# tayloraswift/jpeg

Measured on AMD Instinct MI355X. Metric: Mpixels/s decode (IDCT+dequant+upsample+YCbCr->RGB); % HBM roofline, higher is better.
Workload: dtype f32; 1 GPU; C3: one 8192x8192 ycc8 4:2:0 image per GPU per step, fused Spectral->RGB8 decode (ring of 4 distinct images); sampling=4:2:0, output=RGB8, coefficients=distribution N (SURVEY 8d), seeded, quanta=CompressionLevel luminance/chrominance(1.0), parallelism=independent images x1 (weak scaling), no data-path collective

## Files before the change

include/jpeg_amd.h:

```cpp
#ifndef JPEG_AMD_H
#define JPEG_AMD_H

#include <stddef.h>
#include <stdint.h>

#ifdef __cplusplus
extern "C" {
#endif

#define JPEG_AMD_VERSION 100
#define JPEG_AMD_MAX_PLANES 4

typedef enum jpeg_amd_status {
    JPEG_AMD_OK      = 0,
    JPEG_AMD_EINVAL  = -1,
    JPEG_AMD_ENOMEM  = -2,
    JPEG_AMD_EHIP    = -3,
    JPEG_AMD_ENODEV  = -4,
    JPEG_AMD_ENOSUP  = -5
} jpeg_amd_status;

typedef struct jpeg_amd_ctx jpeg_amd_ctx;

typedef struct jpeg_amd_layout {
// ... 5 lines not shown
    int32_t factor_y[JPEG_AMD_MAX_PLANES];
    int32_t units_x[JPEG_AMD_MAX_PLANES];
    int32_t units_y[JPEG_AMD_MAX_PLANES];
    int32_t qi[JPEG_AMD_MAX_PLANES];
} jpeg_amd_layout;

typedef enum jpeg_amd_color {
    JPEG_AMD_COLOR_YCC8 = 0,
    JPEG_AMD_COLOR_RGB8 = 1
} jpeg_amd_color;

int         jpeg_amd_version(void);
const char *jpeg_amd_strerror(int status);
int         jpeg_amd_device_count(int *count);
#define JPEG_AMD_CTX_OWN_STREAM 1
int         jpeg_amd_ctx_create(int device, void *stream, int flags, jpeg_amd_ctx **ctx);
int         jpeg_amd_ctx_destroy(jpeg_amd_ctx *ctx);
int         jpeg_amd_ctx_synchronize(jpeg_amd_ctx *ctx);
int         jpeg_amd_last_hip_error(const jpeg_amd_ctx *ctx);
int         jpeg_amd_layout_units(jpeg_amd_layout *layout);

int jpeg_amd_malloc(jpeg_amd_ctx *ctx, size_t bytes, void **d_ptr);
int jpeg_amd_free(jpeg_amd_ctx *ctx, void *d_ptr);
int jpeg_amd_memcpy_h2d(jpeg_amd_ctx *ctx, void *d_dst, const void *h_src, size_t bytes);
int jpeg_amd_memcpy_d2h(jpeg_amd_ctx *ctx, void *h_dst, const void *d_src, size_t bytes);
int jpeg_amd_timer_begin(jpeg_amd_ctx *ctx);
int jpeg_amd_timer_end(jpeg_amd_ctx *ctx, float *elapsed_ms);


int jpeg_amd_idct_plane(jpeg_amd_ctx *ctx, const int16_t *d_coef, int units_x, int units_y,
                        const uint16_t h_quanta_zigzag[64], int precision,
                        uint16_t *d_plane);

int jpeg_amd_spectral_idct(jpeg_amd_ctx *ctx, const jpeg_amd_layout *layout,
// ... 257 lines not shown
```

jpeg_amd/_lib.py:

```python
from __future__ import annotations

import ctypes as C
import os

HERE = os.path.dirname(os.path.abspath(__file__))
LIB_PATH = os.environ.get("JPEG_AMD_LIBRARY") or os.path.join(HERE, "libjpeg_amd.so")
MAX_PLANES = 4

OK, EINVAL, ENOMEM, EHIP, ENODEV, ENOSUP = 0, -1, -2, -3, -4, -5
COLOR_YCC8, COLOR_RGB8 = 0, 1
CTX_OWN_STREAM = 1


class JpegAmdError(RuntimeError):
    def __init__(self, status: int, what: str, hip: int = 0):
        self.status, self.hip = status, hip
        msg = lib().jpeg_amd_strerror(status).decode()
        super().__init__(f"{what}: {msg} (status {status}" + (f", hipError {hip})" if hip else ")"))


class Layout(C.Structure):
    _fields_ = [
        ("width", C.c_int32), ("height", C.c_int32), ("precision", C.c_int32),
        ("nplanes", C.c_int32), ("scale_x", C.c_int32), ("scale_y", C.c_int32),
        ("factor_x", C.c_int32 * MAX_PLANES), ("factor_y", C.c_int32 * MAX_PLANES),
        ("units_x", C.c_int32 * MAX_PLANES), ("units_y", C.c_int32 * MAX_PLANES),
# ... 2 lines not shown


_p = C.c_void_p
_pp = C.POINTER(C.c_void_p)
_szp = C.POINTER(C.c_size_t)
_L = C.POINTER(Layout)

SIGNATURES = {
    "jpeg_amd_version": (C.c_int, []),
    "jpeg_amd_strerror": (C.c_char_p, [C.c_int]),
    "jpeg_amd_device_count": (C.c_int, [C.POINTER(C.c_int)]),
    "jpeg_amd_ctx_create": (C.c_int, [C.c_int, _p, C.c_int, _pp]),
    "jpeg_amd_ctx_destroy": (C.c_int, [_p]),
    "jpeg_amd_ctx_synchronize": (C.c_int, [_p]),
    "jpeg_amd_last_hip_error": (C.c_int, [_p]),
    "jpeg_amd_layout_units": (C.c_int, [_L]),
    "jpeg_amd_malloc": (C.c_int, [_p, C.c_size_t, _pp]),
    "jpeg_amd_free": (C.c_int, [_p, _p]),
    "jpeg_amd_memcpy_h2d": (C.c_int, [_p, _p, _p, C.c_size_t]),
    "jpeg_amd_memcpy_d2h": (C.c_int, [_p, _p, _p, C.c_size_t]),
    "jpeg_amd_timer_begin": (C.c_int, [_p]),
    "jpeg_amd_timer_end": (C.c_int, [_p, C.POINTER(C.c_float)]),
    "jpeg_amd_idct_plane": (C.c_int, [_p, _p, C.c_int, C.c_int, _p, C.c_int, _p]),
    "jpeg_amd_spectral_idct": (C.c_int, [_p, _L, _pp, _p, C.c_int, _pp]),
    "jpeg_amd_planar_interleaved": (C.c_int, [_p, _L, _pp, C.c_int, _p]),
    "jpeg_amd_rectangular_unpack": (C.c_int, [_p, _p, C.c_size_t, C.c_int, C.c_int, _p]),
    "jpeg_amd_decode_batch": (C.c_int, [_p, _L, C.c_int, _pp, _szp, _p, C.c_size_t, C.c_int,
                                        C.c_int, C.c_int, _p, C.c_size_t]),
    "jpeg_amd_decode": (C.c_int, [_p, _L, _pp, _p, C.c_int, C.c_int, C.c_int, _p]),
    "jpeg_amd_spectral_rectangular_batch": (C.c_int, [_p, _L, C.c_int, _pp, _szp, _p, C.c_size_t, C.c_int, C.c_int, _p, C.c_size_t]),
# ... 138 lines not shown
```

jpeg_amd/api.py:

```python
from __future__ import annotations

import ctypes as C
from dataclasses import dataclass
from typing import Dict, List, Optional, Sequence, Tuple

import numpy as np

from . import _lib

MAX_PLANES = _lib.MAX_PLANES


class YCbCr:
    code = _lib.COLOR_YCC8


class RGB:
    code = _lib.COLOR_RGB8


def _torch():
    import torch
    return torch


class Context:

    def __init__(self, device: int = 0, stream: Optional[int] = None, own_stream: bool = False):
        torch = _torch()
        if not torch.cuda.is_available():
            raise RuntimeError("jpeg_amd needs a GPU: torch.cuda.is_available() is False "
                               "(there is no CPU fallback)")
        self.device = int(device)
        self.torch_device = torch.device("cuda", self.device)
        if stream is None:
            stream = torch.cuda.current_stream(self.torch_device).cuda_stream
        self._h = C.c_void_p()
        flags = _lib.CTX_OWN_STREAM if own_stream else 0
        _lib.check(_lib.lib().jpeg_amd_ctx_create(self.device, C.c_void_p(stream), flags,
                                                 C.byref(self._h)), "jpeg_amd_ctx_create")

    @property
    def handle(self):
        return self._h

    def synchronize(self):
        _lib.check(_lib.lib().jpeg_amd_ctx_synchronize(self._h), "synchronize", self._h)

    def timer_begin(self):
        _lib.check(_lib.lib().jpeg_amd_timer_begin(self._h), "timer_begin", self._h)

    def timer_end(self) -> float:
        ms = C.c_float()
        _lib.check(_lib.lib().jpeg_amd_timer_end(self._h, C.byref(ms)), "timer_end", self._h)
        return ms.value

    def empty(self, n: int, dtype):
        torch = _torch()
        return torch.empty(max(int(n), 0), dtype=dtype, device=self.torch_device)

    def upload(self, a: np.ndarray):
        torch = _torch()
# ... 700 lines not shown
```

jpeg_amd/csrc/capi.hip:

```cpp
#pragma clang fp contract(off)

#include <hip/hip_runtime.h>

#include <cstdio>
#include <cstdlib>
#include <cstring>
#include <new>
#include <algorithm>
#include <atomic>
#include <memory>
#include <chrono>
#include <system_error>
#include <thread>
#include <vector>

#include "interleave.hpp"
#include "kernels.hpp"
#include "transform.hpp"
#include "worker_pool.hpp"

using namespace jpeg_amd;

struct jpeg_amd_ctx {
    int device = 0;
    hipStream_t stream = nullptr;
    bool own_stream = false;
    hipEvent_t ev_begin = nullptr, ev_end = nullptr;
    void *scratch = nullptr;
    size_t scratch_bytes = 0;
    uint16_t *d_qstage = nullptr;
    uint32_t *d_walk = nullptr;
    int32_t *d_flag = nullptr;
    void *d_region = nullptr;
    size_t region_bytes = 0;
    int qslot = 0;
    int last_hip = 0;
    void *file_pinned[2] = {nullptr, nullptr};
    void *file_device = nullptr;
    size_t file_pinned_bytes = 0, file_device_bytes = 0;
    hipEvent_t file_done[2] = {nullptr, nullptr};
    hipEvent_t file_decoded[2] = {nullptr, nullptr};
// ... 22 lines not shown
    catch (...) { return JPEG_AMD_ENOMEM; }

#define JA_TRY(expr)                          \
    do {                                      \
        const int s_ = (expr);                \
        if (s_ != JPEG_AMD_OK) return s_;     \
    } while (0)

int bind(jpeg_amd_ctx *ctx)
{
    if (!ctx) return JPEG_AMD_EINVAL;
    JA_HIP(ctx, hipSetDevice(ctx->device));
    return JPEG_AMD_OK;
}

int units_of(int size, int stride) { return size / stride + (size % stride != 0 ? 1 : 0); }

int check_layout(const jpeg_amd_layout *L, int ntables)
{
    if (!L) return JPEG_AMD_EINVAL;
    if (L->width <= 0 || L->height <= 0) return JPEG_AMD_EINVAL;
    if (L->precision < 1 || L->precision > 16) return JPEG_AMD_EINVAL;
    if (L->nplanes < 1 || L->nplanes > JPEG_AMD_MAX_PLANES) return JPEG_AMD_EINVAL;
    if (L->scale_x < 1 || L->scale_y < 1) return JPEG_AMD_EINVAL;
    for (int p = 0; p < L->nplanes; ++p) {
        if (L->factor_x[p] < 1 || L->factor_y[p] < 1) return JPEG_AMD_EINVAL;
        if (L->factor_x[p] > L->scale_x || L->factor_y[p] > L->scale_y) return JPEG_AMD_EINVAL;
        if (L->units_x[p] < 0 || L->units_y[p] < 0) return JPEG_AMD_EINVAL;
        if ((long long)L->units_x[p] * L->units_y[p] > (1LL << 30)) return JPEG_AMD_EINVAL;
        if (ntables >= 0 && (L->qi[p] < 0 || L->qi[p] >= ntables)) return JPEG_AMD_EINVAL;
// ... 13 lines not shown
            if (ix >= 8LL * L->units_x[p] || iy >= 8LL * L->units_y[p]) return JPEG_AMD_EINVAL;
        }
    }
    return JPEG_AMD_OK;
}

size_t plane_samples(const jpeg_amd_layout *L, int p)
{
    return (size_t)64 * L->units_x[p] * L->units_y[p];
}

int ensure_scratch(jpeg_amd_ctx *ctx, size_t bytes)
{
    if (bytes <= ctx->scratch_bytes) return JPEG_AMD_OK;
    if (ctx->scratch) {
        JA_HIP(ctx, hipStreamSynchronize(ctx->stream));
        JA_HIP(ctx, hipFree(ctx->scratch));
        ctx->scratch = nullptr;
        ctx->scratch_bytes = 0;
    }
    const size_t want = bytes + bytes / 8 + 4096;
    JA_HIP(ctx, hipMalloc(&ctx->scratch, want));
    ctx->scratch_bytes = want;
    return JPEG_AMD_OK;
}

int stage_quanta(jpeg_amd_ctx *ctx, const uint16_t *h_quanta, int ntables, const uint16_t **d_out)
{
    if (!h_quanta || ntables < 1 || ntables > JPEG_AMD_MAX_PLANES) return JPEG_AMD_EINVAL;
    uint16_t *slot = ctx->d_qstage + (size_t)ctx->qslot * kQSlotElems;
    ctx->qslot = (ctx->qslot + 1) % kQSlots;
// ... 118 lines not shown
struct SparseBudget {
    size_t blocks, arena, elems;
    bool ok;
};
SparseBudget sparse_budget(const jpeg_amd_layout &L)
{
    size_t blocks = 0;
    for (int c = 0; c < L.nplanes; ++c) blocks += (size_t)L.units_x[c] * L.units_y[c];
    const size_t arena = 24 * blocks;
    return {blocks, arena, blocks + arena, blocks + arena < 0xffffffffull};
}

int ensure_file_staging(jpeg_amd_ctx *ctx, size_t slot_bytes)
{
    if (ctx->file_pinned_bytes < slot_bytes) {
        JA_HIP(ctx, hipStreamSynchronize(ctx->stream));
        for (int i = 0; i < 2; ++i) {
            if (ctx->file_pinned[i]) { (void)hipHostFree(ctx->file_pinned[i]); ctx->file_pinned[i] = nullptr; }
            ctx->file_pinned_bytes = 0;
            JA_HIP(ctx, hipHostMalloc(&ctx->file_pinned[i], slot_bytes, hipHostMallocDefault));
            if (!ctx->file_done[i]) JA_HIP(ctx, hipEventCreateWithFlags(&ctx->file_done[i], hipEventDisableTiming));
            if (!ctx->file_decoded[i]) JA_HIP(ctx, hipEventCreateWithFlags(&ctx->file_decoded[i], hipEventDisableTiming));
            if (!ctx->file_fetched[i]) JA_HIP(ctx, hipEventCreateWithFlags(&ctx->file_fetched[i], hipEventDisableTiming));
        }
        ctx->file_pinned_bytes = slot_bytes;
    }
    if (!ctx->file_d2h) JA_HIP(ctx, hipStreamCreateWithFlags(&ctx->file_d2h, hipStreamNonBlocking));
    if (ctx->file_device_bytes < 2 * slot_bytes) {
        JA_HIP(ctx, hipStreamSynchronize(ctx->stream));
        JA_HIP(ctx, hipStreamSynchronize(ctx->file_d2h));
        if (ctx->file_device) { (void)hipFree(ctx->file_device); ctx->file_device = nullptr; ctx->file_device_bytes = 0; }
        JA_HIP(ctx, hipMalloc(&ctx->file_device, 2 * slot_bytes));
        ctx->file_device_bytes = 2 * slot_bytes;
    }
    return JPEG_AMD_OK;
}

int default_host_threads()
{
    int n = (int)std::max(1u, std::thread::hardware_concurrency());
    auto read_two = [](const char *path, long long &a, long long &b) -> bool {
        FILE *f = std::fopen(path, "r");
        if (!f) return false;
        char first[32] = {0};
// ... 82 lines not shown
    if (!ctx) return JPEG_AMD_ENOMEM;
    ctx->device = device;
    int status = JPEG_AMD_OK;
    do {
        if (hipSetDevice(device) != hipSuccess) { status = JPEG_AMD_ENODEV; break; }
        if (flags & JPEG_AMD_CTX_OWN_STREAM) {
            if (hipStreamCreateWithFlags(&ctx->stream, hipStreamNonBlocking) != hipSuccess) { status = JPEG_AMD_EHIP; break; }
            ctx->own_stream = true;
        } else {
            ctx->stream = static_cast<hipStream_t>(stream);
        }
        if (hipEventCreate(&ctx->ev_begin) != hipSuccess || hipEventCreate(&ctx->ev_end) != hipSuccess) { status = JPEG_AMD_EHIP; break; }
        if (hipMalloc(reinterpret_cast<void **>(&ctx->d_qstage), kQSlots * kQSlotElems * sizeof(uint16_t)) != hipSuccess) { status = JPEG_AMD_ENOMEM; break; }
        if (hipMalloc(reinterpret_cast<void **>(&ctx->d_walk), 256) != hipSuccess) { status = JPEG_AMD_ENOMEM; break; }
        if (hipMemset(ctx->d_walk, 0, 256) != hipSuccess) { status = JPEG_AMD_EHIP; break; }
    } while (0);
    if (status != JPEG_AMD_OK) {
        jpeg_amd_ctx_destroy(ctx);
        return status;
    }
    *out = ctx;
    return JPEG_AMD_OK;
}

int jpeg_amd_ctx_destroy(jpeg_amd_ctx *ctx)
{
    if (!ctx) return JPEG_AMD_OK;
    (void)hipSetDevice(ctx->device);
    (void)hipStreamSynchronize(ctx->stream);
    ctx->workers.reset();
    ctx->copiers.reset();
    if (ctx->scratch) (void)hipFree(ctx->scratch);
    if (ctx->d_region) (void)hipFree(ctx->d_region);
    if (ctx->d_qstage) (void)hipFree(ctx->d_qstage);
    if (ctx->d_walk) (void)hipFree(ctx->d_walk);
    if (ctx->d_flag) (void)hipFree(ctx->d_flag);
    for (int i = 0; i < 2; ++i) {
        if (ctx->file_pinned[i]) (void)hipHostFree(ctx->file_pinned[i]);
        if (ctx->file_done[i]) (void)hipEventDestroy(ctx->file_done[i]);
        if (ctx->file_decoded[i]) (void)hipEventDestroy(ctx->file_decoded[i]);
        if (ctx->file_fetched[i]) (void)hipEventDestroy(ctx->file_fetched[i]);
    }
    if (ctx->file_d2h) (void)hipStreamDestroy(ctx->file_d2h);
    if (ctx->file_device) (void)hipFree(ctx->file_device);
    if (ctx->ev_begin) (void)hipEventDestroy(ctx->ev_begin);
    if (ctx->ev_end) (void)hipEventDestroy(ctx->ev_end);
    if (ctx->own_stream && ctx->stream) (void)hipStreamDestroy(ctx->stream);
    delete ctx;
    return JPEG_AMD_OK;
}

int jpeg_amd_ctx_synchronize(jpeg_amd_ctx *ctx)
{
    JA_TRY(bind(ctx));
    JA_HIP(ctx, hipStreamSynchronize(ctx->stream));
    return JPEG_AMD_OK;
}

int jpeg_amd_last_hip_error(const jpeg_amd_ctx *ctx) { return ctx ? ctx->last_hip : 0; }

int jpeg_amd_layout_units(jpeg_amd_layout *L)
{
    if (!L || L->nplanes < 1 || L->nplanes > JPEG_AMD_MAX_PLANES || L->scale_x < 1 ||
        L->scale_y < 1 || L->width <= 0 || L->height <= 0)
        return JPEG_AMD_EINVAL;
    for (int p = 0; p < L->nplanes; ++p) {
        if (L->factor_x[p] < 1 || L->factor_y[p] < 1) return JPEG_AMD_EINVAL;
        L->units_x[p] = units_of(L->width * L->factor_x[p], 8 * L->scale_x);
        L->units_y[p] = units_of(L->height * L->factor_y[p], 8 * L->scale_y);
    }
    return JPEG_AMD_OK;
}


int jpeg_amd_malloc(jpeg_amd_ctx *ctx, size_t bytes, void **d_ptr)
{
    JA_TRY(bind(ctx));
    if (!d_ptr) return JPEG_AMD_EINVAL;
    *d_ptr = nullptr;
    if (bytes == 0) return JPEG_AMD_OK;
    JA_HIP(ctx, hipMalloc(d_ptr, bytes));
    return JPEG_AMD_OK;
}

int jpeg_amd_free(jpeg_amd_ctx *ctx, void *d_ptr)
{
    JA_TRY(bind(ctx));
    if (!d_ptr) return JPEG_AMD_OK;
    JA_HIP(ctx, hipStreamSynchronize(ctx->stream));
    JA_HIP(ctx, hipFree(d_ptr));
    return JPEG_AMD_OK;
}

int jpeg_amd_memcpy_h2d(jpeg_amd_ctx *ctx, void *d_dst, const void *h_src, size_t bytes)
{
    JA_TRY(bind(ctx));
    if (bytes == 0) return JPEG_AMD_OK;
    if (!d_dst || !h_src) return JPEG_AMD_EINVAL;
    JA_HIP(ctx, hipMemcpyAsync(d_dst, h_src, bytes, hipMemcpyHostToDevice, ctx->stream));
    JA_HIP(ctx, hipStreamSynchronize(ctx->stream));
    return JPEG_AMD_OK;
}

int jpeg_amd_memcpy_d2h(jpeg_amd_ctx *ctx, void *h_dst, const void *d_src, size_t bytes)
{
    JA_TRY(bind(ctx));
    if (bytes == 0) return JPEG_AMD_OK;
    if (!h_dst || !d_src) return JPEG_AMD_EINVAL;
    JA_HIP(ctx, hipMemcpyAsync(h_dst, d_src, bytes, hipMemcpyDeviceToHost, ctx->stream));
    JA_HIP(ctx, hipStreamSynchronize(ctx->stream));
    return JPEG_AMD_OK;
}

int jpeg_amd_timer_begin(jpeg_amd_ctx *ctx)
{
    JA_TRY(bind(ctx));
    JA_HIP(ctx, hipEventRecord(ctx->ev_begin, ctx->stream));
    return JPEG_AMD_OK;
}

int jpeg_amd_timer_end(jpeg_amd_ctx *ctx, float *elapsed_ms)
{
    JA_TRY(bind(ctx));
    if (!elapsed_ms) return JPEG_AMD_EINVAL;
    JA_HIP(ctx, hipEventRecord(ctx->ev_end, ctx->stream));
// ... 76 lines not shown
                          const uint16_t *d_quanta, size_t quanta_stride, int ntables,
                          int cosited, jpeg_amd_color color, uint8_t *d_pixels,
                          size_t pixel_stride)
{
    JA_TRY(bind(ctx));
    JA_TRY(check_layout(L, ntables));
    JA_TRY(check_planes_cover_image(L));
    JA_TRY(check_batch8(L, n_images, color));
    if (n_images == 0) return JPEG_AMD_OK;
    if (!d_coef || !coef_stride || !d_quanta || !d_pixels) return JPEG_AMD_EINVAL;
    PlaneSet cs;
    JA_TRY(plane_set(L, d_coef, coef_stride, true, &cs));
    const QuantaRef q{d_quanta, quanta_stride};
    const bool rgb = color == JPEG_AMD_COLOR_RGB8;
    if (fused_decode_supported(*L, cosited != 0)) {
        JA_HIP(ctx, launch_fused_decode(ctx->stream, n_images, *L, cs, q, rgb, ctx->d_walk, d_pixels, pixel_stride));
        return JPEG_AMD_OK;
    }
    return staged_decode(ctx, L, n_images, cs, q, cosited != 0, true, rgb ? PixelKind::RGB8 : PixelKind::YCC8, d_pixels, pixel_stride);
}

int jpeg_amd_decode(jpeg_amd_ctx *ctx, const jpeg_amd_layout *L, const int16_t *const d_coef[],
                    const uint16_t *h_quanta, int ntables, int cosited, jpeg_amd_color color,
                    uint8_t *d_pixels)
{
    JA_TRY(bind(ctx));
    JA_TRY(check_layout(L, ntables));
    const uint16_t *d_q = nullptr;
    JA_TRY(stage_quanta(ctx, h_quanta, ntables, &d_q));
    const size_t zero[JPEG_AMD_MAX_PLANES] = {0, 0, 0, 0};
    return jpeg_amd_decode_batch(ctx, L, 1, d_coef, zero, d_q, 0, ntables, cosited, color,
// ... 16 lines not shown

int stage_regions(jpeg_amd_ctx *ctx, const jpeg_amd_region *h, int n, const int32_t **d_regions, const uint32_t **d_tiles,
                  uint32_t *nwg)
{
    const size_t bytes = (size_t)16 * n + 4 * ((size_t)n + 1);
    std::vector<uint32_t> buf(bytes / 4);
    uint32_t acc = 0;
    for (int i = 0; i < n; ++i) {
        std::memcpy(&buf[4 * (size_t)i], &h[i], 16);
        buf[4 * (size_t)n + i] = acc;
        acc += region_tiles(h[i]);
    }
    buf[4 * (size_t)n + n] = acc;
    if (bytes > ctx->region_bytes) {
        if (ctx->d_region) {
            JA_HIP(ctx, hipStreamSynchronize(ctx->stream));
            JA_HIP(ctx, hipFree(ctx->d_region));
            ctx->d_region = nullptr;
            ctx->region_bytes = 0;
        }
        const size_t want = bytes + bytes / 8 + 4096;
        JA_HIP(ctx, hipMalloc(&ctx->d_region, want));
        ctx->region_bytes = want;
    }
    JA_HIP(ctx, hipMemcpyAsync(ctx->d_region, buf.data(), bytes, hipMemcpyHostToDevice, ctx->stream));
    *d_regions = static_cast<const int32_t *>(ctx->d_region);
    *d_tiles = reinterpret_cast<const uint32_t *>(static_cast<const int32_t *>(ctx->d_region) + 4 * (size_t)n);
    *nwg = acc;
    return JPEG_AMD_OK;
}

// ... 378 lines not shown
    const uint16_t *d_q = nullptr;
    JA_TRY(stage_quanta(ctx, h_quanta, ntables, &d_q));
    const size_t zero[JPEG_AMD_MAX_PLANES] = {0, 0, 0, 0};
    return jpeg_amd_encode_batch(ctx, L, 1, d_pixels, 0, color, d_q, 0, ntables, d_coef, zero);
}


namespace {

struct DeviceBag {
    jpeg_amd_ctx *ctx;
    std::vector<void *> ptrs;
    explicit DeviceBag(jpeg_amd_ctx *c) : ctx(c) {}
    ~DeviceBag()
    {
        (void)hipStreamSynchronize(ctx->stream);
        for (void *p : ptrs) (void)hipFree(p);
    }
    int alloc(size_t bytes, void **out)
    {
        *out = nullptr;
        if (bytes == 0) bytes = 16;
        const hipError_t e = hipMalloc(out, bytes);
        if (e != hipSuccess) { ctx->last_hip = (int)e; return JPEG_AMD_ENOMEM; }
        ptrs.push_back(*out);
        return JPEG_AMD_OK;
    }
    int upload(const void *h, size_t bytes, void **out)
    {
        JA_TRY(alloc(bytes, out));
        if (bytes == 0) return JPEG_AMD_OK;
// ... 20 lines not shown
try {
    JA_TRY(bind(ctx));
    JA_TRY(check_layout(L, ntables));
    if (!h_coef || !h_planes) return JPEG_AMD_EINVAL;
    DeviceBag bag(ctx);
    const int16_t *d_coef[JPEG_AMD_MAX_PLANES] = {};
    uint16_t *d_planes[JPEG_AMD_MAX_PLANES] = {};
    for (int p = 0; p < L->nplanes; ++p) {
        const size_t n = plane_samples(L, p);
        JA_TRY(bag.upload(h_coef[p], n * 2, (void **)&d_coef[p]));
        JA_TRY(bag.alloc(n * 2, (void **)&d_planes[p]));
    }
    JA_TRY(jpeg_amd_spectral_idct(ctx, L, d_coef, h_quanta, ntables, d_planes));
    for (int p = 0; p < L->nplanes; ++p)
        JA_TRY(bag.download(h_planes[p], d_planes[p], plane_samples(L, p) * 2));
    JA_HIP(ctx, hipStreamSynchronize(ctx->stream));
    return JPEG_AMD_OK;
}
JA_NOTHROW_TAIL

int jpeg_amd_host_planar_interleaved(jpeg_amd_ctx *ctx, const jpeg_amd_layout *L,
                                     const uint16_t *const h_planes[], int cosited,
                                     uint16_t *h_rect)
try {
    JA_TRY(bind(ctx));
    JA_TRY(check_layout(L, -1));
    if (!h_planes || !h_rect) return JPEG_AMD_EINVAL;
    DeviceBag bag(ctx);
    const uint16_t *d_planes[JPEG_AMD_MAX_PLANES] = {};
    for (int p = 0; p < L->nplanes; ++p)
        JA_TRY(bag.upload(h_planes[p], plane_samples(L, p) * 2, (void **)&d_planes[p]));
    uint16_t *d_rect = nullptr;
    JA_TRY(bag.alloc(rect_samples(L) * 2, (void **)&d_rect));
    JA_TRY(jpeg_amd_planar_interleaved(ctx, L, d_planes, cosited, d_rect));
    JA_TRY(bag.download(h_rect, d_rect, rect_samples(L) * 2));
    JA_HIP(ctx, hipStreamSynchronize(ctx->stream));
    return JPEG_AMD_OK;
}
JA_NOTHROW_TAIL

int jpeg_amd_host_rectangular_unpack(jpeg_amd_ctx *ctx, const uint16_t *h_rect, size_t npixels,
                                     int nplanes, jpeg_amd_color color, uint8_t *h_pixels)
try {
    JA_TRY(bind(ctx));
    if (nplanes != 1 && nplanes != 3) return JPEG_AMD_EINVAL;
    DeviceBag bag(ctx);
    uint16_t *d_rect = nullptr;
    uint8_t *d_px = nullptr;
    JA_TRY(bag.upload(h_rect, npixels * nplanes * 2, (void **)&d_rect));
    JA_TRY(bag.alloc(npixels * 3, (void **)&d_px));
    JA_TRY(jpeg_amd_rectangular_unpack(ctx, d_rect, npixels, nplanes, color, d_px));
    JA_TRY(bag.download(h_pixels, d_px, npixels * 3));
    JA_HIP(ctx, hipStreamSynchronize(ctx->stream));
    return JPEG_AMD_OK;
}
JA_NOTHROW_TAIL

int jpeg_amd_host_decode(jpeg_amd_ctx *ctx, const jpeg_amd_layout *L,
                         const int16_t *const h_coef[], const uint16_t *h_quanta, int ntables,
                         int cosited, jpeg_amd_color color, uint8_t *h_pixels)
try {
    JA_TRY(bind(ctx));
    JA_TRY(check_layout(L, ntables));
    if (!h_coef || !h_pixels) return JPEG_AMD_EINVAL;
    DeviceBag bag(ctx);
    const int16_t *d_coef[JPEG_AMD_MAX_PLANES] = {};
    for (int p = 0; p < L->nplanes; ++p)
        JA_TRY(bag.upload(h_coef[p], plane_samples(L, p) * 2, (void **)&d_coef[p]));
    uint8_t *d_px = nullptr;
    const size_t nbytes = (size_t)L->width * L->height * 3;
    JA_TRY(bag.alloc(nbytes, (void **)&d_px));
    JA_TRY(jpeg_amd_decode(ctx, L, d_coef, h_quanta, ntables, cosited, color, d_px));
    JA_TRY(bag.download(h_pixels, d_px, nbytes));
    JA_HIP(ctx, hipStreamSynchronize(ctx->stream));
    return JPEG_AMD_OK;
}
JA_NOTHROW_TAIL

int jpeg_amd_host_spectral_rectangular(jpeg_amd_ctx *ctx, const jpeg_amd_layout *L,
                                       const int16_t *const h_coef[], const uint16_t *h_quanta, int ntables,
                                       int cosited, uint16_t *h_rect)
try {
    JA_TRY(bind(ctx));
    JA_TRY(check_layout(L, ntables));
    if (!h_coef || !h_rect) return JPEG_AMD_EINVAL;
    DeviceBag bag(ctx);
    const int16_t *d_coef[JPEG_AMD_MAX_PLANES] = {};
    for (int p = 0; p < L->nplanes; ++p)
        JA_TRY(bag.upload(h_coef[p], plane_samples(L, p) * 2, (void **)&d_coef[p]));
    uint16_t *d_rect = nullptr;
    JA_TRY(bag.alloc(rect_samples(L) * 2, (void **)&d_rect));
    JA_TRY(jpeg_amd_spectral_rectangular(ctx, L, d_coef, h_quanta, ntables, cosited, d_rect));
    JA_TRY(bag.download(h_rect, d_rect, rect_samples(L) * 2));
    JA_HIP(ctx, hipStreamSynchronize(ctx->stream));
    return JPEG_AMD_OK;
}
JA_NOTHROW_TAIL

int jpeg_amd_host_rectangular_spectral(jpeg_amd_ctx *ctx, const jpeg_amd_layout *L, const uint16_t *h_rect,
                                       const uint16_t *h_quanta, int ntables, int16_t *const h_coef[])
try {
    JA_TRY(bind(ctx));
    JA_TRY(check_layout(L, ntables));
    if (!h_rect || !h_coef) return JPEG_AMD_EINVAL;
    DeviceBag bag(ctx);
    uint16_t *d_rect = nullptr;
    JA_TRY(bag.upload(h_rect, rect_samples(L) * 2, (void **)&d_rect));
    int16_t *d_coef[JPEG_AMD_MAX_PLANES] = {};
    for (int p = 0; p < L->nplanes; ++p) JA_TRY(bag.alloc(plane_samples(L, p) * 2, (void **)&d_coef[p]));
    JA_TRY(jpeg_amd_rectangular_spectral(ctx, L, d_rect, h_quanta, ntables, d_coef));
    for (int p = 0; p < L->nplanes; ++p) JA_TRY(bag.download(h_coef[p], d_coef[p], plane_samples(L, p) * 2));
    JA_HIP(ctx, hipStreamSynchronize(ctx->stream));
    return JPEG_AMD_OK;
}
JA_NOTHROW_TAIL

int jpeg_amd_host_rectangular_pack(jpeg_amd_ctx *ctx, const uint8_t *h_pixels, size_t npixels,
                                   int nplanes, jpeg_amd_color color, uint16_t *h_rect)
try {
    JA_TRY(bind(ctx));
    if (nplanes != 1 && nplanes != 3) return JPEG_AMD_EINVAL;
    DeviceBag bag(ctx);
    uint16_t *d_rect = nullptr;
    uint8_t *d_px = nullptr;
    JA_TRY(bag.upload(h_pixels, npixels * 3, (void **)&d_px));
    JA_TRY(bag.alloc(npixels * nplanes * 2, (void **)&d_rect));
    JA_TRY(jpeg_amd_rectangular_pack(ctx, d_px, npixels, nplanes, color, d_rect));
    JA_TRY(bag.download(h_rect, d_rect, npixels * nplanes * 2));
    JA_HIP(ctx, hipStreamSynchronize(ctx->stream));
    return JPEG_AMD_OK;
}
JA_NOTHROW_TAIL

int jpeg_amd_host_rectangular_decomposed(jpeg_amd_ctx *ctx, const jpeg_amd_layout *L,
                                         const uint16_t *h_rect, uint16_t *const h_planes[])
try {
    JA_TRY(bind(ctx));
    JA_TRY(check_layout(L, -1));
    if (!h_rect || !h_planes) return JPEG_AMD_EINVAL;
    DeviceBag bag(ctx);
    uint16_t *d_rect = nullptr;
    JA_TRY(bag.upload(h_rect, rect_samples(L) * 2, (void **)&d_rect));
    uint16_t *d_planes[JPEG_AMD_MAX_PLANES] = {};
    for (int p = 0; p < L->nplanes; ++p)
        JA_TRY(bag.alloc(plane_samples(L, p) * 2, (void **)&d_planes[p]));
    JA_TRY(jpeg_amd_rectangular_decomposed(ctx, L, d_rect, d_planes));
    for (int p = 0; p < L->nplanes; ++p)
        JA_TRY(bag.download(h_planes[p], d_planes[p], plane_samples(L, p) * 2));
    JA_HIP(ctx, hipStreamSynchronize(ctx->stream));
    return JPEG_AMD_OK;
}
JA_NOTHROW_TAIL

int jpeg_amd_host_planar_fdct(jpeg_amd_ctx *ctx, const jpeg_amd_layout *L,
                              const uint16_t *const h_planes[], const uint16_t *h_quanta,
                              int ntables, int16_t *const h_coef[])
try {
    JA_TRY(bind(ctx));
    JA_TRY(check_layout(L, ntables));
    if (!h_coef || !h_planes) return JPEG_AMD_EINVAL;
    DeviceBag bag(ctx);
    const uint16_t *d_planes[JPEG_AMD_MAX_PLANES] = {};
    int16_t *d_coef[JPEG_AMD_MAX_PLANES] = {};
    for (int p = 0; p < L->nplanes; ++p) {
        const size_t n = plane_samples(L, p);
        JA_TRY(bag.upload(h_planes[p], n * 2, (void **)&d_planes[p]));
        JA_TRY(bag.alloc(n * 2, (void **)&d_coef[p]));
    }
    JA_TRY(jpeg_amd_planar_fdct(ctx, L, d_planes, h_quanta, ntables, d_coef));
    for (int p = 0; p < L->nplanes; ++p)
        JA_TRY(bag.download(h_coef[p], d_coef[p], plane_samples(L, p) * 2));
    JA_HIP(ctx, hipStreamSynchronize(ctx->stream));
    return JPEG_AMD_OK;
}
JA_NOTHROW_TAIL

int jpeg_amd_host_encode(jpeg_amd_ctx *ctx, const jpeg_amd_layout *L, const uint8_t *h_pixels,
                         jpeg_amd_color color, const uint16_t *h_quanta, int ntables,
                         int16_t *const h_coef[])
try {
    JA_TRY(bind(ctx));
    JA_TRY(check_layout(L, ntables));
    if (!h_coef || !h_pixels) return JPEG_AMD_EINVAL;
    DeviceBag bag(ctx);
    uint8_t *d_px = nullptr;
    JA_TRY(bag.upload(h_pixels, (size_t)L->width * L->height * 3, (void **)&d_px));
    int16_t *d_coef[JPEG_AMD_MAX_PLANES] = {};
    for (int p = 0; p < L->nplanes; ++p)
        JA_TRY(bag.alloc(plane_samples(L, p) * 2, (void **)&d_coef[p]));
    JA_TRY(jpeg_amd_encode(ctx, L, d_px, color, h_quanta, ntables, d_coef));
    for (int p = 0; p < L->nplanes; ++p)
        JA_TRY(bag.download(h_coef[p], d_coef[p], plane_samples(L, p) * 2));
    JA_HIP(ctx, hipStreamSynchronize(ctx->stream));
    return JPEG_AMD_OK;
}
JA_NOTHROW_TAIL

int jpeg_amd_decompress(jpeg_amd_ctx *ctx, const uint8_t *h_jpeg, size_t nbytes, int cosited,
                        jpeg_amd_color color, uint8_t *h_pixels, size_t pixel_capacity,
                        jpeg_amd_frame_info *info_out)
try {
    JA_TRY(bind(ctx));
    if (!h_jpeg) return JPEG_AMD_EINVAL;
    jpeg_amd_frame_info fi;
    JA_TRY(jpeg_amd_jpeg_inspect(h_jpeg, nbytes, &fi));
    if (info_out) *info_out = fi;
    if (fi.precision != 8 || (fi.ncomponents != 1 && fi.ncomponents != 3)) return JPEG_AMD_ENOSUP;
    const size_t need = (size_t)fi.width * fi.height * 3;
// ... 200 lines not shown
            }
            JA_HIP(ctx, hipStreamWaitEvent(ctx->file_d2h, ctx->file_decoded[slot], 0));
            if (!direct_out) JA_HIP(ctx, hipMemcpyAsync(host + px_off, dev + px_off, npx * m, hipMemcpyDeviceToHost, ctx->file_d2h));
            else if (pixel_stride == npx) JA_HIP(ctx, hipMemcpyAsync(h_pixels + (size_t)base * npx, dev + px_off, npx * m, hipMemcpyDeviceToHost, ctx->file_d2h));
            else
                for (int i = 0; i < m; ++i)
                    JA_HIP(ctx, hipMemcpyAsync(h_pixels + (size_t)(base + i) * pixel_stride, dev + px_off + npx * i, npx, hipMemcpyDeviceToHost, ctx->file_d2h));
            JA_HIP(ctx, hipEventRecord(ctx->file_done[slot], ctx->file_d2h));
            return JPEG_AMD_OK;
        };
        result = submit();
        if (result != JPEG_AMD_OK) break;
        if (k >= 1 && copies_out) begin_drain(k - 1);
    }
    { const int ds = end_drain(); if (result == JPEG_AMD_OK) result = ds; }
    if (result != JPEG_AMD_OK) { (void)hipStreamSynchronize(ctx->stream); (void)hipStreamSynchronize(ctx->file_d2h); return result; }
    JA_HIP(ctx, wait_event(ctx->file_done[(nchunks - 1) & 1]));
    if (copies_out) { begin_drain(nchunks - 1); JA_TRY(end_drain()); }
    return JPEG_AMD_OK;
}

}

int jpeg_amd_decompress_batch(jpeg_amd_ctx *ctx, const uint8_t *const h_jpeg[], const size_t nbytes[],
                              int n_images, int nthreads, int cosited, jpeg_amd_color color,
                              uint8_t *h_pixels, size_t pixel_stride, jpeg_amd_frame_info *info_out)
try {
    if (!h_pixels) return JPEG_AMD_EINVAL;
    return decompress_batch_impl(ctx, h_jpeg, nbytes, n_images, nthreads, cosited, color, h_pixels, nullptr, pixel_stride, info_out);
}
JA_NOTHROW_TAIL
// ... 187 lines not shown
            }
        }, nthreads);
        const int fetched_status = fetch_chunk >= 0 ? fetch(fetch_chunk) : JPEG_AMD_OK;
        pool.finish();
        if (fetched_status != JPEG_AMD_OK) return fetched_status;
        for (int st : status) if (st != JPEG_AMD_OK) return st;
        return JPEG_AMD_OK;
    };
    int result = host_region(-1, 0, -1);
    if (result == JPEG_AMD_OK) result = submit(0);
    for (int k = 0; k < nchunks && result == JPEG_AMD_OK; ++k) {
        result = host_region(k - 1, k + 1, k);
        if (result == JPEG_AMD_OK && k + 1 < nchunks) result = submit(k + 1);
    }
    if (result == JPEG_AMD_OK) result = host_region(nchunks - 1, nchunks, -1);
    if (result != JPEG_AMD_OK) { (void)hipStreamSynchronize(ctx->stream); (void)hipStreamSynchronize(ctx->file_d2h); }
    return result;
}

}

int jpeg_amd_compress_batch(jpeg_amd_ctx *ctx, jpeg_amd_frame_info *frame, const uint8_t *h_pixels,
                            size_t pixel_stride, int n_images, jpeg_amd_color color,
                            const int32_t *quanta_key, const uint16_t *h_quanta, const int32_t *h_quanta_keys,
                            int ntables, const jpeg_amd_scan *scans, int nscans,
                            const jpeg_amd_metadata *metadata, int nmetadata, int nthreads,
                            uint8_t *h_out, size_t out_stride, size_t nbytes[])
try {
    if (!h_pixels) return JPEG_AMD_EINVAL;
    return compress_batch_impl(ctx, frame, h_pixels, nullptr, pixel_stride, n_images, color, quanta_key, h_quanta, h_quanta_keys, ntables,
                               scans, nscans, metadata, nmetadata, nthreads, h_out, out_stride, nbytes);
// ... 103 lines not shown
                                const int16_t *const d_coef_in[], const uint16_t *h_quanta, int ntables,
                                const uint16_t *h_quanta_out, int16_t *const d_coef_out[])
{
    JA_TRY(bind(ctx));
    JA_TRY(check_layout(L, ntables));
    const uint16_t *d_q = nullptr, *d_qo = nullptr;
    JA_TRY(stage_quanta(ctx, h_quanta, ntables, &d_q));
    if (h_quanta_out) JA_TRY(stage_quanta(ctx, h_quanta_out, ntables, &d_qo));
    if (!ctx->d_flag) JA_HIP(ctx, hipMalloc(reinterpret_cast<void **>(&ctx->d_flag), 256));
    JA_HIP(ctx, hipMemsetAsync(ctx->d_flag, 0, sizeof(int32_t), ctx->stream));
    const size_t zero[JPEG_AMD_MAX_PLANES] = {0, 0, 0, 0};
    JA_TRY(jpeg_amd_spectral_transform_batch(ctx, L, 1, op, region, d_coef_in, zero, d_q, 0, ntables, d_qo, d_coef_out, zero,
                                             ctx->d_flag));
    int32_t flag = 0;
    JA_HIP(ctx, hipMemcpyAsync(&flag, ctx->d_flag, sizeof flag, hipMemcpyDeviceToHost, ctx->stream));
    JA_HIP(ctx, hipStreamSynchronize(ctx->stream));
    return flag ? JPEG_AMD_EINVAL : JPEG_AMD_OK;
}

int jpeg_amd_transform(jpeg_amd_ctx *ctx, const uint8_t *h_jpeg, size_t nbytes, int op, const jpeg_amd_region *region,
                       const uint16_t *h_requant, int nthreads, uint8_t *h_out, size_t capacity, size_t *nbytes_out,
                       jpeg_amd_frame_info *out_info)
try {
    JA_TRY(bind(ctx));
    if (!h_jpeg || !nbytes_out || op < 0 || op > 7) return JPEG_AMD_EINVAL;
    jpeg_amd_frame_info fi;
    JA_TRY(jpeg_amd_jpeg_inspect(h_jpeg, nbytes, &fi));
    const int nc = fi.ncomponents;
    if (nc < 1 || nc > JPEG_AMD_MAX_PLANES) return JPEG_AMD_ENOSUP;
    int nscans = 0, nmeta = 0;
    int32_t keys[JPEG_AMD_MAX_PLANES] = {};
// ... 22 lines not shown
    int16_t *ocoef[JPEG_AMD_MAX_PLANES] = {};
    for (int c = 0; c < nc; ++c) {
        outp[c].resize(plane_samples(&O, c));
        ocoef[c] = outp[c].data();
    }
    {
        DeviceBag bag(ctx);
        const int16_t *d_in[JPEG_AMD_MAX_PLANES] = {};
        int16_t *d_out[JPEG_AMD_MAX_PLANES] = {};
        for (int c = 0; c < nc; ++c) {
            JA_TRY(bag.upload(coef[c], plane_samples(&L, c) * 2, (void **)&d_in[c]));
            JA_TRY(bag.alloc(plane_samples(&O, c) * 2, (void **)&d_out[c]));
        }
        JA_TRY(jpeg_amd_spectral_transform(ctx, &L, op, region, d_in, &quanta[0][0], nc, h_requant, d_out));
        for (int c = 0; c < nc; ++c) JA_TRY(bag.download(ocoef[c], d_out[c], plane_samples(&O, c) * 2));
        JA_HIP(ctx, hipStreamSynchronize(ctx->stream));
    }
    std::vector<int32_t> tkeys;
    std::vector<uint16_t> tables;
    for (int c = 0; c < nc; ++c)
        if (std::find(tkeys.begin(), tkeys.end(), keys[c]) == tkeys.end()) tkeys.push_back(keys[c]);
    std::sort(tkeys.begin(), tkeys.end());
    for (int32_t k : tkeys) {
        const int c = (int)(std::find(keys, keys + nc, k) - keys);
        uint16_t t[64];
        if (h_requant) std::memcpy(t, h_requant + 64 * c, sizeof t);
        else JA_TRY(jpeg_amd_transform_quanta(op, quanta[c], t));
        tables.insert(tables.end(), t, t + 64);
    }
    jpeg_amd_frame_info of = fi;
    of.width = O.width; of.height = O.height;
// ... 13 lines not shown
```

Measured before the change: 905,100 Mpixels/s.

## Alternate fused decode launches across two hazard-checked streams

When the context wraps the null stream and the new serial flag is not set, two extra streams are created. Each fused decode launch goes to the next stream in turn, provided its read and write byte ranges do not conflict with work recorded on the other stream. Otherwise it falls back to the main stream and clears the records. The aim is to let consecutive independent decodes overlap, hiding kernel tails and launch gaps. The cost is per-call range bookkeeping, a separate ticket area per stream, and replacing every stream synchronize with a sync over all streams.

```diff
diff --git a/include/jpeg_amd.h b/include/jpeg_amd.h
--- a/include/jpeg_amd.h
+++ b/include/jpeg_amd.h
@@ -43,10 +43,12 @@
 const char *jpeg_amd_strerror(int status);
 int         jpeg_amd_device_count(int *count);
 #define JPEG_AMD_CTX_OWN_STREAM 1
+#define JPEG_AMD_CTX_SERIAL 2
 int         jpeg_amd_ctx_create(int device, void *stream, int flags, jpeg_amd_ctx **ctx);
 int         jpeg_amd_ctx_destroy(jpeg_amd_ctx *ctx);
 int         jpeg_amd_ctx_synchronize(jpeg_amd_ctx *ctx);
 int         jpeg_amd_last_hip_error(const jpeg_amd_ctx *ctx);
+int         jpeg_amd_ctx_last_lane(const jpeg_amd_ctx *ctx);
 int         jpeg_amd_layout_units(jpeg_amd_layout *layout);
 
 int jpeg_amd_malloc(jpeg_amd_ctx *ctx, size_t bytes, void **d_ptr);
diff --git a/jpeg_amd/_lib.py b/jpeg_amd/_lib.py
--- a/jpeg_amd/_lib.py
+++ b/jpeg_amd/_lib.py
@@ -9,7 +9,7 @@
 
 OK, EINVAL, ENOMEM, EHIP, ENODEV, ENOSUP = 0, -1, -2, -3, -4, -5
 COLOR_YCC8, COLOR_RGB8 = 0, 1
-CTX_OWN_STREAM = 1
+CTX_OWN_STREAM, CTX_SERIAL = 1, 2
 
 
 class JpegAmdError(RuntimeError):
@@ -42,6 +42,7 @@
     "jpeg_amd_ctx_destroy": (C.c_int, [_p]),
     "jpeg_amd_ctx_synchronize": (C.c_int, [_p]),
     "jpeg_amd_last_hip_error": (C.c_int, [_p]),
+    "jpeg_amd_ctx_last_lane": (C.c_int, [_p]),
     "jpeg_amd_layout_units": (C.c_int, [_L]),
     "jpeg_amd_malloc": (C.c_int, [_p, C.c_size_t, _pp]),
     "jpeg_amd_free": (C.c_int, [_p, _p]),
diff --git a/jpeg_amd/api.py b/jpeg_amd/api.py
--- a/jpeg_amd/api.py
+++ b/jpeg_amd/api.py
@@ -26,7 +26,7 @@
 
 class Context:
 
-    def __init__(self, device: int = 0, stream: Optional[int] = None, own_stream: bool = False):
+    def __init__(self, device: int = 0, stream: Optional[int] = None, own_stream: bool = False, serial: bool = False):
         torch = _torch()
         if not torch.cuda.is_available():
             raise RuntimeError("jpeg_amd needs a GPU: torch.cuda.is_available() is False "
@@ -36,7 +36,7 @@
         if stream is None:
             stream = torch.cuda.current_stream(self.torch_device).cuda_stream
         self._h = C.c_void_p()
-        flags = _lib.CTX_OWN_STREAM if own_stream else 0
+        flags = (_lib.CTX_OWN_STREAM if own_stream else 0) | (_lib.CTX_SERIAL if serial else 0)
         _lib.check(_lib.lib().jpeg_amd_ctx_create(self.device, C.c_void_p(stream), flags,
                                                  C.byref(self._h)), "jpeg_amd_ctx_create")
 
@@ -46,6 +46,9 @@
 
     def synchronize(self):
         _lib.check(_lib.lib().jpeg_amd_ctx_synchronize(self._h), "synchronize", self._h)
+
+    def last_lane(self) -> int:
+        return int(_lib.lib().jpeg_amd_ctx_last_lane(self._h))
 
     def timer_begin(self):
         _lib.check(_lib.lib().jpeg_amd_timer_begin(self._h), "timer_begin", self._h)
diff --git a/jpeg_amd/csrc/capi.hip b/jpeg_amd/csrc/capi.hip
--- a/jpeg_amd/csrc/capi.hip
+++ b/jpeg_amd/csrc/capi.hip
@@ -21,10 +21,35 @@
 
 using namespace jpeg_amd;
 
+struct ByteRange {
+    uintptr_t lo, hi;
+    bool meets(const ByteRange &o) const { return lo < o.hi && o.lo < hi; }
+};
+struct LaneRecord {
+    static constexpr int kMax = 48;
+    ByteRange read[kMax], written[kMax];
+    int nread = 0, nwritten = 0;
+    void clear() { nread = nwritten = 0; }
+    static bool covered(const ByteRange *set, int n, const ByteRange &r)
+    {
+        for (int i = 0; i < n; ++i) if (set[i].lo <= r.lo && r.hi <= set[i].hi) return true;
+        return false;
+    }
+    static bool any_meets(const ByteRange *set, int n, const ByteRange &r)
+    {
+        for (int i = 0; i < n; ++i) if (set[i].meets(r)) return true;
+        return false;
+    }
+};
+
 struct jpeg_amd_ctx {
     int device = 0;
     hipStream_t stream = nullptr;
     bool own_stream = false;
+    hipStream_t lane[2] = {nullptr, nullptr};
+    LaneRecord lane_record[2];
+    int next_lane = 0;
+    int last_lane = -1;
     hipEvent_t ev_begin = nullptr, ev_end = nullptr;
     void *scratch = nullptr;
     size_t scratch_bytes = 0;
@@ -77,6 +102,44 @@
     return JPEG_AMD_OK;
 }
 
+hipError_t sync_all(jpeg_amd_ctx *ctx)
+{
+    for (int i = 0; i < 2; ++i) {
+        if (!ctx->lane[i]) continue;
+        const hipError_t e = hipStreamSynchronize(ctx->lane[i]);
+        if (e != hipSuccess) return e;
+        ctx->lane_record[i].clear();
+    }
+    return hipStreamSynchronize(ctx->stream);
+}
+
+hipStream_t choose_lane(jpeg_amd_ctx *ctx, const ByteRange *reads, int nreads, const ByteRange &written, uint32_t **tickets)
+{
+    *tickets = ctx->d_walk;
+    ctx->last_lane = -1;
+    if (!ctx->lane[0]) return ctx->stream;
+    const int mine = ctx->next_lane;
+    LaneRecord &own = ctx->lane_record[mine];
+    const LaneRecord &other = ctx->lane_record[mine ^ 1];
+    bool ok = !LaneRecord::any_meets(other.written, other.nwritten, written) && !LaneRecord::any_meets(other.read, other.nread, written);
+    for (int i = 0; ok && i < nreads; ++i) ok = !LaneRecord::any_meets(other.written, other.nwritten, reads[i]);
+    int new_reads = 0;
+    for (int i = 0; i < nreads; ++i) new_reads += !LaneRecord::covered(own.read, own.nread, reads[i]);
+    const bool new_write = !LaneRecord::covered(own.written, own.nwritten, written);
+    if (!ok || own.nread + new_reads > LaneRecord::kMax || own.nwritten + (new_write ? 1 : 0) > LaneRecord::kMax) {
+        ctx->lane_record[0].clear();
+        ctx->lane_record[1].clear();
+        return ctx->stream;
+    }
+    for (int i = 0; i < nreads; ++i)
+        if (!LaneRecord::covered(own.read, own.nread, reads[i])) own.read[own.nread++] = reads[i];
+    if (new_write) own.written[own.nwritten++] = written;
+    ctx->next_lane = mine ^ 1;
+    ctx->last_lane = mine;
+    *tickets = ctx->d_walk + 32 + 16 * mine;
+    return ctx->lane[mine];
+}
+
 int units_of(int size, int stride) { return size / stride + (size % stride != 0 ? 1 : 0); }
 
 int check_layout(const jpeg_amd_layout *L, int ntables)
@@ -120,7 +183,7 @@
 {
     if (bytes <= ctx->scratch_bytes) return JPEG_AMD_OK;
     if (ctx->scratch) {
-        JA_HIP(ctx, hipStreamSynchronize(ctx->stream));
+        JA_HIP(ctx, sync_all(ctx));
         JA_HIP(ctx, hipFree(ctx->scratch));
         ctx->scratch = nullptr;
         ctx->scratch_bytes = 0;
@@ -269,7 +332,7 @@
 int ensure_file_staging(jpeg_amd_ctx *ctx, size_t slot_bytes)
 {
     if (ctx->file_pinned_bytes < slot_bytes) {
-        JA_HIP(ctx, hipStreamSynchronize(ctx->stream));
+        JA_HIP(ctx, sync_all(ctx));
         for (int i = 0; i < 2; ++i) {
             if (ctx->file_pinned[i]) { (void)hipHostFree(ctx->file_pinned[i]); ctx->file_pinned[i] = nullptr; }
             ctx->file_pinned_bytes = 0;
@@ -282,7 +345,7 @@
     }
     if (!ctx->file_d2h) JA_HIP(ctx, hipStreamCreateWithFlags(&ctx->file_d2h, hipStreamNonBlocking));
     if (ctx->file_device_bytes < 2 * slot_bytes) {
-        JA_HIP(ctx, hipStreamSynchronize(ctx->stream));
+        JA_HIP(ctx, sync_all(ctx));
         JA_HIP(ctx, hipStreamSynchronize(ctx->file_d2h));
         if (ctx->file_device) { (void)hipFree(ctx->file_device); ctx->file_device = nullptr; ctx->file_device_bytes = 0; }
         JA_HIP(ctx, hipMalloc(&ctx->file_device, 2 * slot_bytes));
@@ -395,6 +458,11 @@
         if (hipMalloc(reinterpret_cast<void **>(&ctx->d_qstage), kQSlots * kQSlotElems * sizeof(uint16_t)) != hipSuccess) { status = JPEG_AMD_ENOMEM; break; }
         if (hipMalloc(reinterpret_cast<void **>(&ctx->d_walk), 256) != hipSuccess) { status = JPEG_AMD_ENOMEM; break; }
         if (hipMemset(ctx->d_walk, 0, 256) != hipSuccess) { status = JPEG_AMD_EHIP; break; }
+        if (!ctx->stream && !(flags & JPEG_AMD_CTX_SERIAL)) {
+            for (int i = 0; i < 2 && status == JPEG_AMD_OK; ++i)
+                if (hipStreamCreateWithFlags(&ctx->lane[i], hipStreamDefault) != hipSuccess) { ctx->lane[i] = nullptr; status = JPEG_AMD_EHIP; }
+            if (status != JPEG_AMD_OK) break;
+        }
     } while (0);
     if (status != JPEG_AMD_OK) {
         jpeg_amd_ctx_destroy(ctx);
@@ -408,7 +476,7 @@
 {
     if (!ctx) return JPEG_AMD_OK;
     (void)hipSetDevice(ctx->device);
-    (void)hipStreamSynchronize(ctx->stream);
+    (void)sync_all(ctx);
     ctx->workers.reset();
     ctx->copiers.reset();
     if (ctx->scratch) (void)hipFree(ctx->scratch);
@@ -426,6 +494,7 @@
     if (ctx->file_device) (void)hipFree(ctx->file_device);
     if (ctx->ev_begin) (void)hipEventDestroy(ctx->ev_begin);
     if (ctx->ev_end) (void)hipEventDestroy(ctx->ev_end);
+    for (int i = 0; i < 2; ++i) if (ctx->lane[i]) (void)hipStreamDestroy(ctx->lane[i]);
     if (ctx->own_stream && ctx->stream) (void)hipStreamDestroy(ctx->stream);
     delete ctx;
     return JPEG_AMD_OK;
@@ -434,11 +503,13 @@
 int jpeg_amd_ctx_synchronize(jpeg_amd_ctx *ctx)
 {
     JA_TRY(bind(ctx));
-    JA_HIP(ctx, hipStreamSynchronize(ctx->stream));
+    JA_HIP(ctx, sync_all(ctx));
     return JPEG_AMD_OK;
 }
 
 int jpeg_amd_last_hip_error(const jpeg_amd_ctx *ctx) { return ctx ? ctx->last_hip : 0; }
+
+int jpeg_amd_ctx_last_lane(const jpeg_amd_ctx *ctx) { return ctx ? ctx->last_lane : -1; }
 
 int jpeg_amd_layout_units(jpeg_amd_layout *L)
 {
@@ -468,7 +539,7 @@
 {
     JA_TRY(bind(ctx));
     if (!d_ptr) return JPEG_AMD_OK;
-    JA_HIP(ctx, hipStreamSynchronize(ctx->stream));
+    JA_HIP(ctx, sync_all(ctx));
     JA_HIP(ctx, hipFree(d_ptr));
     return JPEG_AMD_OK;
 }
@@ -479,7 +550,7 @@
     if (bytes == 0) return JPEG_AMD_OK;
     if (!d_dst || !h_src) return JPEG_AMD_EINVAL;
     JA_HIP(ctx, hipMemcpyAsync(d_dst, h_src, bytes, hipMemcpyHostToDevice, ctx->stream));
-    JA_HIP(ctx, hipStreamSynchronize(ctx->stream));
+    JA_HIP(ctx, sync_all(ctx));
     return JPEG_AMD_OK;
 }
 
@@ -489,7 +560,7 @@
     if (bytes == 0) return JPEG_AMD_OK;
     if (!h_dst || !d_src) return JPEG_AMD_EINVAL;
     JA_HIP(ctx, hipMemcpyAsync(h_dst, d_src, bytes, hipMemcpyDeviceToHost, ctx->stream));
-    JA_HIP(ctx, hipStreamSynchronize(ctx->stream));
+    JA_HIP(ctx, sync_all(ctx));
     return JPEG_AMD_OK;
 }
 
@@ -596,7 +667,19 @@
     const QuantaRef q{d_quanta, quanta_stride};
     const bool rgb = color == JPEG_AMD_COLOR_RGB8;
     if (fused_decode_supported(*L, cosited != 0)) {
-        JA_HIP(ctx, launch_fused_decode(ctx->stream, n_images, *L, cs, q, rgb, ctx->d_walk, d_pixels, pixel_stride));
+        ByteRange reads[JPEG_AMD_MAX_PLANES + 1];
+        int nreads = 0;
+        const size_t last = (size_t)n_images - 1;
+        for (int p = 0; p < L->nplanes; ++p) {
+            const uintptr_t lo = reinterpret_cast<uintptr_t>(d_coef[p]);
+            reads[nreads++] = ByteRange{lo, lo + (last * coef_stride[p] + plane_samples(L, p)) * sizeof(int16_t)};
+        }
+        const uintptr_t q_lo = reinterpret_cast<uintptr_t>(d_quanta), px_lo = reinterpret_cast<uintptr_t>(d_pixels);
+        reads[nreads++] = ByteRange{q_lo, q_lo + (last * quanta_stride + (size_t)ntables * 64) * sizeof(uint16_t)};
+        const ByteRange written{px_lo, px_lo + last * pixel_stride + (size_t)3 * L->width * L->height};
+        uint32_t *tickets = nullptr;
+        const hipStream_t stream = choose_lane(ctx, reads, nreads, written, &tickets);
+        JA_HIP(ctx, launch_fused_decode(stream, n_images, *L, cs, q, rgb, tickets, d_pixels, pixel_stride));
         return JPEG_AMD_OK;
     }
     return staged_decode(ctx, L, n_images, cs, q, cosited != 0, true, rgb ? PixelKind::RGB8 : PixelKind::YCC8, d_pixels, pixel_stride);
@@ -643,7 +726,7 @@
     buf[4 * (size_t)n + n] = acc;
     if (bytes > ctx->region_bytes) {
         if (ctx->d_region) {
-            JA_HIP(ctx, hipStreamSynchronize(ctx->stream));
+            JA_HIP(ctx, sync_all(ctx));
             JA_HIP(ctx, hipFree(ctx->d_region));
             ctx->d_region = nullptr;
             ctx->region_bytes = 0;
@@ -1052,7 +1135,7 @@
     explicit DeviceBag(jpeg_amd_ctx *c) : ctx(c) {}
     ~DeviceBag()
     {
-        (void)hipStreamSynchronize(ctx->stream);
+        (void)sync_all(ctx);
         for (void *p : ptrs) (void)hipFree(p);
     }
     int alloc(size_t bytes, void **out)
@@ -1103,7 +1186,7 @@
     JA_TRY(jpeg_amd_spectral_idct(ctx, L, d_coef, h_quanta, ntables, d_planes));
     for (int p = 0; p < L->nplanes; ++p)
         JA_TRY(bag.download(h_planes[p], d_planes[p], plane_samples(L, p) * 2));
-    JA_HIP(ctx, hipStreamSynchronize(ctx->stream));
+    JA_HIP(ctx, sync_all(ctx));
     return JPEG_AMD_OK;
 }
 JA_NOTHROW_TAIL
@@ -1123,7 +1206,7 @@
     JA_TRY(bag.alloc(rect_samples(L) * 2, (void **)&d_rect));
     JA_TRY(jpeg_amd_planar_interleaved(ctx, L, d_planes, cosited, d_rect));
     JA_TRY(bag.download(h_rect, d_rect, rect_samples(L) * 2));
-    JA_HIP(ctx, hipStreamSynchronize(ctx->stream));
+    JA_HIP(ctx, sync_all(ctx));
     return JPEG_AMD_OK;
 }
 JA_NOTHROW_TAIL
@@ -1140,7 +1223,7 @@
     JA_TRY(bag.alloc(npixels * 3, (void **)&d_px));
     JA_TRY(jpeg_amd_rectangular_unpack(ctx, d_rect, npixels, nplanes, color, d_px));
     JA_TRY(bag.download(h_pixels, d_px, npixels * 3));
-    JA_HIP(ctx, hipStreamSynchronize(ctx->stream));
+    JA_HIP(ctx, sync_all(ctx));
     return JPEG_AMD_OK;
 }
 JA_NOTHROW_TAIL
@@ -1161,7 +1244,7 @@
     JA_TRY(bag.alloc(nbytes, (void **)&d_px));
     JA_TRY(jpeg_amd_decode(ctx, L, d_coef, h_quanta, ntables, cosited, color, d_px));
     JA_TRY(bag.download(h_pixels, d_px, nbytes));
-    JA_HIP(ctx, hipStreamSynchronize(ctx->stream));
+    JA_HIP(ctx, sync_all(ctx));
     return JPEG_AMD_OK;
 }
 JA_NOTHROW_TAIL
@@ -1181,7 +1264,7 @@
     JA_TRY(bag.alloc(rect_samples(L) * 2, (void **)&d_rect));
     JA_TRY(jpeg_amd_spectral_rectangular(ctx, L, d_coef, h_quanta, ntables, cosited, d_rect));
     JA_TRY(bag.download(h_rect, d_rect, rect_samples(L) * 2));
-    JA_HIP(ctx, hipStreamSynchronize(ctx->stream));
+    JA_HIP(ctx, sync_all(ctx));
     return JPEG_AMD_OK;
 }
 JA_NOTHROW_TAIL
@@ -1199,7 +1282,7 @@
     for (int p = 0; p < L->nplanes; ++p) JA_TRY(bag.alloc(plane_samples(L, p) * 2, (void **)&d_coef[p]));
     JA_TRY(jpeg_amd_rectangular_spectral(ctx, L, d_rect, h_quanta, ntables, d_coef));
     for (int p = 0; p < L->nplanes; ++p) JA_TRY(bag.download(h_coef[p], d_coef[p], plane_samples(L, p) * 2));
-    JA_HIP(ctx, hipStreamSynchronize(ctx->stream));
+    JA_HIP(ctx, sync_all(ctx));
     return JPEG_AMD_OK;
 }
 JA_NOTHROW_TAIL
@@ -1216,7 +1299,7 @@
     JA_TRY(bag.alloc(npixels * nplanes * 2, (void **)&d_rect));
     JA_TRY(jpeg_amd_rectangular_pack(ctx, d_px, npixels, nplanes, color, d_rect));
     JA_TRY(bag.download(h_rect, d_rect, npixels * nplanes * 2));
-    JA_HIP(ctx, hipStreamSynchronize(ctx->stream));
+    JA_HIP(ctx, sync_all(ctx));
     return JPEG_AMD_OK;
 }
 JA_NOTHROW_TAIL
@@ -1236,7 +1319,7 @@
     JA_TRY(jpeg_amd_rectangular_decomposed(ctx, L, d_rect, d_planes));
     for (int p = 0; p < L->nplanes; ++p)
         JA_TRY(bag.download(h_planes[p], d_planes[p], plane_samples(L, p) * 2));
-    JA_HIP(ctx, hipStreamSynchronize(ctx->stream));
+    JA_HIP(ctx, sync_all(ctx));
     return JPEG_AMD_OK;
 }
 JA_NOTHROW_TAIL
@@ -1259,7 +1342,7 @@
     JA_TRY(jpeg_amd_planar_fdct(ctx, L, d_planes, h_quanta, ntables, d_coef));
     for (int p = 0; p < L->nplanes; ++p)
         JA_TRY(bag.download(h_coef[p], d_coef[p], plane_samples(L, p) * 2));
-    JA_HIP(ctx, hipStreamSynchronize(ctx->stream));
+    JA_HIP(ctx, sync_all(ctx));
     return JPEG_AMD_OK;
 }
 JA_NOTHROW_TAIL
@@ -1280,7 +1363,7 @@
     JA_TRY(jpeg_amd_encode(ctx, L, d_px, color, h_quanta, ntables, d_coef));
     for (int p = 0; p < L->nplanes; ++p)
         JA_TRY(bag.download(h_coef[p], d_coef[p], plane_samples(L, p) * 2));
-    JA_HIP(ctx, hipStreamSynchronize(ctx->stream));
+    JA_HIP(ctx, sync_all(ctx));
     return JPEG_AMD_OK;
 }
 JA_NOTHROW_TAIL
@@ -1511,7 +1594,7 @@
         if (k >= 1 && copies_out) begin_drain(k - 1);
     }
     { const int ds = end_drain(); if (result == JPEG_AMD_OK) result = ds; }
-    if (result != JPEG_AMD_OK) { (void)hipStreamSynchronize(ctx->stream); (void)hipStreamSynchronize(ctx->file_d2h); return result; }
+    if (result != JPEG_AMD_OK) { (void)sync_all(ctx); (void)hipStreamSynchronize(ctx->file_d2h); return result; }
     JA_HIP(ctx, wait_event(ctx->file_done[(nchunks - 1) & 1]));
     if (copies_out) { begin_drain(nchunks - 1); JA_TRY(end_drain()); }
     return JPEG_AMD_OK;
@@ -1729,7 +1812,7 @@
         if (result == JPEG_AMD_OK && k + 1 < nchunks) result = submit(k + 1);
     }
     if (result == JPEG_AMD_OK) result = host_region(nchunks - 1, nchunks, -1);
-    if (result != JPEG_AMD_OK) { (void)hipStreamSynchronize(ctx->stream); (void)hipStreamSynchronize(ctx->file_d2h); }
+    if (result != JPEG_AMD_OK) { (void)sync_all(ctx); (void)hipStreamSynchronize(ctx->file_d2h); }
     return result;
 }
 
@@ -1863,7 +1946,7 @@
                                              ctx->d_flag));
     int32_t flag = 0;
     JA_HIP(ctx, hipMemcpyAsync(&flag, ctx->d_flag, sizeof flag, hipMemcpyDeviceToHost, ctx->stream));
-    JA_HIP(ctx, hipStreamSynchronize(ctx->stream));
+    JA_HIP(ctx, sync_all(ctx));
     return flag ? JPEG_AMD_EINVAL : JPEG_AMD_OK;
 }
 
@@ -1916,7 +1999,7 @@
         }
         JA_TRY(jpeg_amd_spectral_transform(ctx, &L, op, region, d_in, &quanta[0][0], nc, h_requant, d_out));
         for (int c = 0; c < nc; ++c) JA_TRY(bag.download(ocoef[c], d_out[c], plane_samples(&O, c) * 2));
-        JA_HIP(ctx, hipStreamSynchronize(ctx->stream));
+        JA_HIP(ctx, sync_all(ctx));
     }
     std::vector<int32_t> tkeys;
     std::vector<uint16_t> tables;
```

Result: faster. 985,900 Mpixels/s (median of 6 runs) (+8.9%).
